# abhi1kumar/SUP-NeRF

Hardware: AMD Instinct MI355X
Metric: rays/sec at 4096 rays x 64 samples (fused render forward) (higher is better)
Workload: dtype f32

## Files before the change

### sup-nerf_amd/csrc/snr_mlp16.hip

```cpp
#include <atomic>

#include "snr_mlp16_core.hpp"
#include "snr_host.hpp"

namespace snr {

struct Epi {
    float lo;
    const float* zlds;
    const float* zglb;
    float hi;
    float* dump;
};
struct EpiRegs { f32x4 z; };

__device__ __forceinline__ uint32_t spread_nibbles(uint32_t m16) {
    return ((m16 >> 12) & 0xFu) | (((m16 >> 8) & 0xFu) << 8) | (((m16 >> 4) & 0xFu) << 16) | ((m16 & 0xFu) << 24);
}

template <bool LATLDS>
__device__ __forceinline__ EpiRegs epi_load(const Epi& c, int T, int g) {
    EpiRegs e;
    e.z = f32x4{0.f, 0.f, 0.f, 0.f};
    if (LATLDS) e.z = *reinterpret_cast<const f32x4*>(c.zlds + 16 * T + 4 * g);
    else if (c.zglb) e.z = *reinterpret_cast<const f32x4*>(c.zglb + 16 * T + 4 * g);
    return e;
}

template <bool MASKS>
__device__ __forceinline__ void epi_value(const f32x4& acc, f32x4& x, const Epi& c, const EpiRegs& e, int r, uint32_t& m16) {
    float v = acc[r];
    if (MASKS) m16 = __builtin_amdgcn_alignbit(m16, __float_as_uint(0.f - v), 31);
    v = __builtin_amdgcn_fmed3f(v, c.lo, c.hi);
    x[r] = v + e.z[r];
    if (MASKS) asm volatile("" : "+v"(m16));
}

template <int NT>
__device__ __forceinline__ void acc_from_bias(f32x4 (&acc)[16], const float* bias , int g) {
#pragma unroll
    for (int t = 0; t < NT; ++t) acc[t] = *reinterpret_cast<const f32x4*>(bias + 16 * t + 4 * g);
}

template <int NT, int WAVES, bool LATLDS, bool MASKS, bool DUMP>
__device__ __forceinline__ void layer_from_acc(f32x4 (&accP)[16], Ring16& ring, float* lds, const float* bias, const Epi& c, int g, const Dma16& dm,
                                               const float* base, bool pre, const f32x4 (&xe)[2], const float* next_first, int next_rows,
                                               uint32_t (&mw)[4]) {
    f32x4 accC[16];
    f32x4 a0, a1;
    constexpr int rows_mid = NT * 16;
    constexpr int chunk_floats = rows_mid * KC;
    if (pre) {
        chunk_dma16<WAVES>(dm, base, lds + (ring.cur ^ 1) * WBUF16, lds, rows_mid);
        const float* wb = lds + ring.cur * WBUF16;
        first_pair(a0, a1, wb + ring.aoff[0]);
        acc_from_bias<NT>(accC, bias, g);
        tile_mma<NT, false>(accC, accP, xe[0], wb + ring.aoff[0], a0, a1, wb + ring.aoff[1]);
        tile_mma<NT, false>(accC, accP, xe[1], wb + ring.aoff[1], a0, a1, nullptr);
        ring_turn(ring);
    } else {
        acc_from_bias<NT>(accC, bias, g);
    }
    constexpr int NG = NT / 2;
    EpiRegs e = epi_load<LATLDS>(c, 0, g);
    f32x4 xa, xb;
    uint32_t m16 = 0u;
#pragma unroll
    for (int r = 3; r >= 0; --r) epi_value<MASKS>(accP[0], xa, c, e, r, m16);
    if (DUMP) *reinterpret_cast<f32x4*>(c.dump) = xa;
#pragma unroll
    for (int ch = 0; ch < 8; ++ch) {
        const float* src = (ch < 7) ? base + (ch + 1) * chunk_floats : next_first;
        const int rows = (ch < 7) ? rows_mid : next_rows;
        float* const dst = lds + (ring.cur ^ 1) * WBUF16;
        const float* wb = lds + ring.cur * WBUF16;
        first_pair(a0, a1, wb + ring.aoff[0]);
        tile_mma<NT, false>(accC, accP, xa, wb + ring.aoff[0], a0, a1, wb + ring.aoff[1], [&](int gi) {
            if (gi == 0) e = epi_load<LATLDS>(c, 2 * ch + 1, g);
            constexpr int PSTEP = (WAVES == 8) ? 2 : 1;
            if (gi % PSTEP == 0 && (gi / PSTEP) * 8 * WAVES < rows) chunk_piece16<WAVES>(dm, src, dst, lds, rows, gi / PSTEP);
#pragma unroll
            for (int k = (gi * 4) / NG; k < ((gi + 1) * 4) / NG; ++k) epi_value<MASKS>(accP[2 * ch + 1], xb, c, e, 3 - k, m16);
            if (DUMP && gi == NG - 1) *reinterpret_cast<f32x4*>(c.dump + 16 * (2 * ch + 1)) = xb;
        });
        if (ch & 1) { mw[ch >> 1] = m16; m16 = 0u; }
        if (ch == 7) {
            tile_mma<NT, true>(accC, accP, xb, wb + ring.aoff[1], a0, a1, nullptr);
        } else {
            tile_mma<NT, false>(accC, accP, xb, wb + ring.aoff[1], a0, a1, nullptr, [&](int gi) {
                if (gi == 0) e = epi_load<LATLDS>(c, 2 * ch + 2, g);
#pragma unroll
                for (int k = (gi * 4) / NG; k < ((gi + 1) * 4) / NG; ++k) epi_value<MASKS>(accP[2 * ch + 2], xa, c, e, 3 - k, m16);
                if (DUMP && gi == NG - 1) *reinterpret_cast<f32x4*>(c.dump + 16 * (2 * ch + 2)) = xa;
            });
        }
        ring_turn(ring);
    }
}

__device__ __forceinline__ void store_masks16x4(uint4* __restrict__ dst , const uint32_t (&mw)[4], int wave, int lane) {
    const int n = lane & 15, g = lane >> 4;
    uint32_t w[4];
#pragma unroll
    for (int i = 0; i < 4; ++i) {
        const uint32_t mine = spread_nibbles(mw[i]) << (4 * (g >> 1));
        w[i] = mine | (uint32_t)__shfl_xor((int)mine, 32, 64);
    }
    if (g < 2) dst[16 * (wave & 1) + n + 32 * g] = make_uint4(w[0], w[1], w[2], w[3]);
}

#ifdef SNR_STAMPS
#define SNR16_STAMP(i) do { if (io.sigmas && lane == 0) { unsigned long long t_; asm volatile("s_memtime %0\n\ts_waitcnt lgkmcnt(0)" : "=s"(t_) :: "memory"); \
        reinterpret_cast<unsigned long long*>(io.sigmas)[(tile_wg * WAVES + wave) * 8 + (i)] = t_; } } while (0)
#define SNR16_STAMP_HWID(i) do { if (io.sigmas && lane == 0) { unsigned a_, b_; asm volatile("s_getreg_b32 %0, hwreg(HW_REG_HW_ID)\n\ts_getreg_b32 %1, hwreg(HW_REG_XCC_ID)" : "=s"(a_), "=s"(b_)); \
        reinterpret_cast<unsigned long long*>(io.sigmas)[(tile_wg * WAVES + wave) * 8 + (i)] = (unsigned long long)a_ | ((unsigned long long)b_ << 32); } } while (0)
#else
#define SNR16_STAMP(i) do {} while (0)
#define SNR16_STAMP_HWID(i) do {} while (0)
#endif

template <int MODE, int WAVES, bool LATLDS, bool MASKS, bool DUMP>
__global__ void __launch_bounds__(WAVES * 64, 2)
decoder_fwd16_kernel(DecoderIO io, Layout L, Lds16 lo, const float* __restrict__ xyz, const float* __restrict__ viewdir, RayGeom gm,
                     float* __restrict__ out_rgb, float* __restrict__ out_depth, float* __restrict__ out_acc) {
    extern __shared__ __attribute__((aligned(16))) float lds[];
    constexpr int WGP = WAVES * 16;
    const int tid = threadIdx.x, lane = tid & 63, wave = tid >> 6, n = lane & 15, g = lane >> 4;
    const long long tile_wg = blockIdx.x;
    const long long gp_raw = tile_wg * WGP + wave * 16 + n;
    const bool live = gp_raw < io.n_points;
    const long long gp = live ? gp_raw : io.n_points - 1;
    const long long tile32 = tile_wg * (WAVES / 2) + (wave >> 1);
    const bool tile_live = tile32 * 32 < io.n_points;
    const int sb = io.sb, tb = io.tb;
    const int n_relu = n_relu_layers(sb, tb);
    SNR16_STAMP(0);
    __builtin_amdgcn_s_setprio(3);
    float px, py, pz, dx, dy, dz, zc = 0.f;
    if (MODE == 0) {
        px = xyz[gp * 3]; py = xyz[gp * 3 + 1]; pz = xyz[gp * 3 + 2];
        dx = viewdir[gp * 3]; dy = viewdir[gp * 3 + 1]; dz = viewdir[gp * 3 + 2];
    } else {
        const PointId id = point_id(gm, tile_wg, WGP, wave * 16 + n, live);
        const SamplePoint sp = make_sample(gm, id.ray, id.s, id.obj);
        px = sp.x; py = sp.y; pz = sp.z; dx = sp.dx; dy = sp.dy; dz = sp.dz; zc = sp.zc;
    }
    const float* bias = lds + lo.bias;
    const float* heads = bias + L.n_mfma_layers * 256;
    const float* zero = lds + lo.zero;
    const float* lat_lane = io.latent + (gp / io.points_per_obj) * (long long)L.n_lat * 256;
    const float* lat_wg = io.latent + ((tile_wg * WGP) / io.points_per_obj) * (long long)L.n_lat * 256;

    Ring16 ring;
    ring.cur = 0;
    Dma16 dm;
    dm.voff = lane * 16u + 4096u;
    dm.lds0 = __builtin_amdgcn_readfirstlane((unsigned)(size_t)(__attribute__((address_space(3))) float*)lds);
    dm.wave = __builtin_amdgcn_readfirstlane(wave);
    {
        const int sw = (n >> 1) & 7;
        ring.aoff[0] = n * KC + (((0 + g) ^ sw) << 2);
        ring.aoff[1] = n * KC + (((4 + g) ^ sw) << 2);
    }
    constexpr long long C256 = 256 * KC;
    const int li_encshape = sb + 1, li_view = sb + 2, li_last = sb + tb + 2;
    const float* const stream = io.packed + L.fwd;
    auto layer_base = [&](int li) { return stream + 2 * C256 + (long long)(li - 1) * 8 * C256 + (li > li_view ? C256 : 0); };
    auto layer_first = [&](int li) { return layer_base(li) + (li == li_view ? 8 * C256 : 0); };
    f32x4 xin[4], xd[2];
    {
        chunk_dma16<WAVES>(dm, stream, lds, lds, 256);
        for (int r = dm.wave; r < L.n_mfma_layers + 3; r += WAVES) row_dma16(dm, io.packed + L.bias + r * 256, lds + lo.bias + r * 256, lds);
        if (LATLDS)
            for (int r = dm.wave; r < L.n_lat; r += WAVES) row_dma16(dm, lat_wg + r * 256, lds + lo.lat + r * 256, lds);
        if (tid < 64) *reinterpret_cast<f32x4*>(lds + lo.zero + 4 * tid) = f32x4{0.f, 0.f, 0.f, 0.f};
        float* sc = lds + lo.scratch + wave * PE_WAVE16 + n * PE_ROW;
#pragma unroll 1
        for (int i = 0; i < 8; i += 2) {
            const int q = 8 * g + i;
            if (q < 3 * XYZ_FREQ) {
                f32x2 sn, cs;
                pe_sincos2(f32x2{ldexpf(pick3(px, py, pz, q % 3), q / 3), ldexpf(pick3(px, py, pz, (q + 1) % 3), (q + 1) / 3)}, &sn, &cs);
                sc[3 + q] = sn[0]; sc[3 + 3 * XYZ_FREQ + q] = cs[0];
                sc[4 + q] = sn[1]; sc[4 + 3 * XYZ_FREQ + q] = cs[1];
            }
        }
        {
            const int q = 3 * g;
            f32x2 sn, cs;
            pe_sincos2(f32x2{ldexpf(pick3(dx, dy, dz, q % 3), q / 3), ldexpf(pick3(dx, dy, dz, (q + 1) % 3), (q + 1) / 3)}, &sn, &cs);
            sc[64 + 3 + q] = sn[0]; sc[64 + 3 + 3 * DIR_FREQ + q] = cs[0];
            sc[64 + 4 + q] = sn[1]; sc[64 + 4 + 3 * DIR_FREQ + q] = cs[1];
            float s1, c1;
            pe_sincos(ldexpf(pick3(dx, dy, dz, (q + 2) % 3), (q + 2) / 3), &s1, &c1);
            sc[64 + 5 + q] = s1; sc[64 + 5 + 3 * DIR_FREQ + q] = c1;
        }
        if (g == 0) {
            sc[0] = px; sc[1] = py; sc[2] = pz; sc[63] = 0.f;
            sc[64] = dx; sc[65] = dy; sc[66] = dz;
#pragma unroll
            for (int f = D_DIR; f < 32; ++f) sc[64 + f] = 0.f;
        }
        asm volatile("s_waitcnt vmcnt(0)" ::: "memory");
        __syncthreads();
#pragma unroll
        for (int T = 0; T < 4; ++T)
#pragma unroll
            for (int r = 0; r < 4; ++r) xin[T][r] = sc[16 * T + 4 * g + r];
#pragma unroll
        for (int T = 0; T < 2; ++T)
#pragma unroll
            for (int r = 0; r < 4; ++r) xd[T][r] = sc[64 + 16 * T + 4 * g + r];
        if (WAVES == 4) __syncthreads();
    }

    __builtin_amdgcn_s_setprio(0);
    SNR16_STAMP(1);
    f32x4 accP[16];
    {
        f32x4 accC[16];
        f32x4 a0, a1;
        acc_from_bias<16>(accC, bias, g);
#pragma unroll
        for (int ch = 0; ch < 2; ++ch) {
            chunk_dma16<WAVES>(dm, ch == 0 ? stream + C256 : layer_first(1), lds + (ring.cur ^ 1) * WBUF16, lds, 256);
            const float* wb = lds + ring.cur * WBUF16;
            first_pair(a0, a1, wb + ring.aoff[0]);
            tile_mma<16, false>(accC, accP, xin[2 * ch], wb + ring.aoff[0], a0, a1, wb + ring.aoff[1]);
            if (ch == 1) tile_mma<16, true>(accC, accP, xin[2 * ch + 1], wb + ring.aoff[1], a0, a1, nullptr);
            else tile_mma<16, false>(accC, accP, xin[2 * ch + 1], wb + ring.aoff[1], a0, a1, nullptr);
            ring_turn(ring);
        }
    }

    SNR16_STAMP(2);
    uint32_t mw[4] = {0u, 0u, 0u, 0u};
    float o_sigma = 0.f;
    float pos_inf = __builtin_inff();
    asm volatile("" : "+v"(pos_inf));
    float* const dump_lane = DUMP ? io.act + gp * 256 + 4 * g : nullptr;
    auto epi_of = [&](int lp) {
        const int la = latent_after(lp, sb, tb);
        Epi c;
        c.lo = (lp != li_encshape) ? 0.f : -__builtin_inff();
        c.zlds = (la >= 0) ? lds + lo.lat + la * 256 : zero;
        c.zglb = (la >= 0) ? lat_lane + la * 256 : nullptr;
        c.hi = pos_inf;
        c.dump = DUMP ? dump_lane + (long long)lp * io.n_points * 256 : nullptr;
        return c;
    };
    auto after_layer_input = [&](int lp) {
        if (MASKS && lp != li_encshape && tile_live) store_masks16x4(io.masks + (tile32 * n_relu + relu_slot(lp, sb)) * 64, mw, wave, lane);
    };
#pragma unroll 1
    for (int li = 1; li <= li_last; ++li) {
        const int lp = li - 1;
        const Epi c = epi_of(lp);
        if (li == li_view) {
            SNR16_STAMP(3);
            float s = 0.f;
#pragma unroll
            for (int T = 0; T < 16; ++T) {
                const f32x4 ws = *reinterpret_cast<const f32x4*>(heads + 16 * T + 4 * g);
#pragma unroll
                for (int r = 0; r < 4; ++r) s = fmaf(ws[r], accP[T][r], s);
            }
            s += __shfl_xor(s, 16, 64);
            s += __shfl_xor(s, 32, 64);
            const float pre = s + heads[L.sigma_b - L.sigma_w];
            o_sigma = pre > 20.f ? pre : log1pf(expf(pre));
        }
        layer_from_acc<16, WAVES, LATLDS, MASKS, DUMP>(accP, ring, lds, bias + li * 256, c, g, dm, layer_base(li), li == li_view, xd, layer_first(li + 1),
                                                       (li == li_last) ? 128 : 256, mw);
        after_layer_input(lp);
    }
    SNR16_STAMP(4);
    {
        const Epi c = epi_of(li_last);
        layer_from_acc<8, WAVES, LATLDS, MASKS, DUMP>(accP, ring, lds, bias + (li_last + 1) * 256, c, g, dm, layer_base(li_last + 1), false, xd, nullptr, 0, mw);
        after_layer_input(li_last);
    }

    SNR16_STAMP(5);
    __builtin_amdgcn_s_setprio(3);
    float o_r, o_g, o_b;
    {
        const float* w2 = heads + (L.rgb2_w - L.sigma_w);
        float pr = 0.f, pg = 0.f, pb = 0.f;
        uint32_t m16 = 0u, mr[4] = {0u, 0u, 0u, 0u};
        float* const dmp = DUMP ? dump_lane + (long long)(li_last + 1) * io.n_points * 256 : nullptr;
#pragma unroll
        for (int T = 0; T < 8; ++T) {
            const f32x4 wr = *reinterpret_cast<const f32x4*>(w2 + 16 * T + 4 * g);
            const f32x4 wg = *reinterpret_cast<const f32x4*>(w2 + 128 + 16 * T + 4 * g);
            const f32x4 wb = *reinterpret_cast<const f32x4*>(w2 + 256 + 16 * T + 4 * g);
            f32x4 xv;
#pragma unroll
            for (int r = 3; r >= 0; --r) {
                float v = accP[T][r];
                m16 = __builtin_amdgcn_alignbit(m16, __float_as_uint(0.f - v), 31);
                v = fmaxf(v, 0.f);
                xv[r] = v;
            }
#pragma unroll
            for (int r = 0; r < 4; ++r) { pr = fmaf(wr[r], xv[r], pr); pg = fmaf(wg[r], xv[r], pg); pb = fmaf(wb[r], xv[r], pb); }
            if (DUMP) *reinterpret_cast<f32x4*>(dmp + 16 * T) = xv;
            if ((T & 3) == 3) { mr[T >> 2] = m16; m16 = 0u; }
        }
        if (MASKS && tile_live) store_masks16x4(io.masks + (tile32 * n_relu + (n_relu - 1)) * 64, mr, wave, lane);
        pr += __shfl_xor(pr, 16, 64); pr += __shfl_xor(pr, 32, 64);
        pg += __shfl_xor(pg, 16, 64); pg += __shfl_xor(pg, 32, 64);
        pb += __shfl_xor(pb, 16, 64); pb += __shfl_xor(pb, 32, 64);
        const float* b2 = heads + (L.rgb2_b - L.sigma_w);
        o_r = pr + b2[0]; o_g = pg + b2[1]; o_b = pb + b2[2];
    }

    SNR16_STAMP_HWID(6);
#ifndef SNR_STAMPS
    if (live && g == 0 && io.sigmas) io.sigmas[gp] = o_sigma;
#endif
    if (live && g == 0) {
        if (io.rgbs) { io.rgbs[gp * 3] = o_r; io.rgbs[gp * 3 + 1] = o_g; io.rgbs[gp * 3 + 2] = o_b; }
    }
    if (MODE == 1) {
        float* comp = lds + lo.comp;
        if (g == 0) {
            float* c = comp + (wave * 16 + n) * COMP_STRIDE;
            c[0] = o_sigma; c[1] = o_r; c[2] = o_g; c[3] = o_b; c[4] = zc;
        }
        __syncthreads();
        const int S = gm.S;
        const int rays_here = WGP / S;
        const bool white = gm.flags & SNR_WHITE_BKGD;
        for (int r = wave; r < rays_here; r += WAVES) {
            const long long ray = tile_wg * rays_here + r;
            if (ray >= gm.n_rays) break;
            const float* c0 = comp + r * S * COMP_STRIDE;
            RayOut o = composite_ray_fwd(S, lane, white, [&](int k, float& s_, float& r_, float& g_, float& b_, float& z_, float& zn_) {
                const float* c = c0 + k * COMP_STRIDE;
                s_ = c[0]; r_ = c[1]; g_ = c[2]; b_ = c[3]; z_ = c[4];
                zn_ = (k < S - 1) ? c[COMP_STRIDE + 4] : 0.f;
            });
            if (lane == 0) {
                out_rgb[ray * 3] = o.r; out_rgb[ray * 3 + 1] = o.g; out_rgb[ray * 3 + 2] = o.b;
                out_depth[ray] = o.depth; out_acc[ray] = o.acc;
            }
        }
    }
    SNR16_STAMP(7);
}

}

using namespace snr;


template <int MODE, int WAVES, bool LATLDS, bool MASKS, bool DUMP>
static int launch16(const DecoderIO& io, const Layout& L, const Lds16& lo, const float* xyz, const float* viewdir, const RayGeom& g, float* rgb,
                    float* depth, float* acc, hipStream_t st) {
    auto kern = decoder_fwd16_kernel<MODE, WAVES, LATLDS, MASKS, DUMP>;
    static std::atomic<uint64_t> granted{0};
    int dev = 0;
    if (hipGetDevice(&dev) != hipSuccess) return SNR_E_LAUNCH;
    const uint64_t bit = dev < 64 ? (uint64_t)1 << dev : 0;
    if (!(granted.load(std::memory_order_acquire) & bit)) {
        if (hipFuncSetAttribute(reinterpret_cast<const void*>(kern), hipFuncAttributeMaxDynamicSharedMemorySize, 160 * 1024) != hipSuccess) return SNR_E_LAUNCH;
        granted.fetch_or(bit, std::memory_order_release);
    }
    const unsigned grid = (unsigned)((io.n_points + WAVES * 16 - 1) / (WAVES * 16));
    kern<<<grid, WAVES * 64, (size_t)lo.total * 4, st>>>(io, L, lo, xyz, viewdir, g, rgb, depth, acc);
    return snr_check_launch_();
}

template <int WAVES>
static int launch16_w(int mode, const DecoderIO& io, const Layout& L, const float* xyz, const float* viewdir, const RayGeom& g, float* rgb,
                      float* depth, float* acc, hipStream_t st) {
    const bool latlds = (io.points_per_obj % (WAVES * 16)) == 0 && L.n_lat <= LDS_LAT_ROWS;
    const bool masks = io.masks != nullptr;
    const Lds16 lo = make_lds16(WAVES, L.n_mfma_layers, latlds ? L.n_lat : LDS_LAT_ROWS + 1);
#define SNR_L16(M, LL, MK, DP) launch16<M, WAVES, LL, MK, DP>(io, L, lo, xyz, viewdir, g, rgb, depth, acc, st)
    if (mode == 0) {
        if (latlds) return masks ? SNR_L16(0, true, true, false) : SNR_L16(0, true, false, false);
        return masks ? SNR_L16(0, false, true, false) : SNR_L16(0, false, false, false);
    }
    if (latlds) return masks ? SNR_L16(1, true, true, false) : SNR_L16(1, true, false, false);
    return masks ? SNR_L16(1, false, true, false) : SNR_L16(1, false, false, false);
#undef SNR_L16
}

int snr_fp32_fwd16_launch_(int mode, const DecoderIO& io, const Layout& L, const float* xyz, const float* viewdir, const RayGeom& g, float* rgb,
                           float* depth, float* acc, void* stream_) {
    hipStream_t st = (hipStream_t)stream_;
    if (io.act) return SNR_E_UNSUPPORTED;
    const bool lat4 = (io.points_per_obj % 64) == 0 && L.n_lat <= LDS_LAT_ROWS;
    const Lds16 lo4 = make_lds16(4, L.n_mfma_layers, lat4 ? L.n_lat : LDS_LAT_ROWS + 1);
    const bool four = lo4.total * 4 <= 80 * 1024 && (mode == 0 || (g.S <= 64 && 64 % g.S == 0));
    return four ? launch16_w<4>(mode, io, L, xyz, viewdir, g, rgb, depth, acc, st) : launch16_w<8>(mode, io, L, xyz, viewdir, g, rgb, depth, acc, st);
}
```

### sup-nerf_amd/csrc/snr_mlp16_core.hpp

```cpp
#pragma once
#include "snr_mlp_core.hpp"

namespace snr {

constexpr int PE_WAVE16 = 16 * PE_ROW;
constexpr int WBUF16 = 256 * KC;

struct Lds16 { int ring1, scratch, comp, bias, lat, zero, total; };
inline Lds16 make_lds16(int waves, int n_mfma_layers, int n_lat) {
    Lds16 o;
    o.ring1 = WBUF16;
    int p = 2 * WBUF16;
    if (waves == 8) { o.scratch = p; p += 8 * PE_WAVE16; o.comp = p; p += 128 * COMP_STRIDE; }
    else { o.scratch = o.ring1; o.comp = 0; }
    p = (p + 3) & ~3;
    o.bias = p; p += (n_mfma_layers + 3) * 256;
    o.lat = p; p += (n_lat <= LDS_LAT_ROWS ? n_lat : 0) * 256;
    o.zero = p; p += 256;
    o.total = p;
    return o;
}

template <int K>
__device__ __forceinline__ void dma_piece_imm(unsigned voff, const void* sbase, unsigned m0v) {
    asm volatile("s_mov_b32 m0, %2\n\ts_nop 0\n\tglobal_load_lds_dwordx4 %0, %1 offset:%3" :: "v"(voff), "s"(sbase), "s"(m0v), "n"(1024 * K - 4096) : "memory");
}
__device__ __forceinline__ void dma_piece(int k, unsigned voff, const void* sbase, unsigned m0v) {
    switch (k) {
        case 0: dma_piece_imm<0>(voff, sbase, m0v); break;
        case 1: dma_piece_imm<1>(voff, sbase, m0v); break;
        case 2: dma_piece_imm<2>(voff, sbase, m0v); break;
        case 3: dma_piece_imm<3>(voff, sbase, m0v); break;
        case 4: dma_piece_imm<4>(voff, sbase, m0v); break;
        case 5: dma_piece_imm<5>(voff, sbase, m0v); break;
        case 6: dma_piece_imm<6>(voff, sbase, m0v); break;
        default: dma_piece_imm<7>(voff, sbase, m0v); break;
    }
}
struct Dma16 {
    unsigned voff;
    unsigned lds0;
    int wave;
};
template <int WAVES>
__device__ __forceinline__ void chunk_piece16(const Dma16& d, const float* __restrict__ g, const float* lds_dst, const float* lds_base, int rows, int i) {
    const unsigned sl = (unsigned)(rows * 128 / WAVES) * (unsigned)d.wave;
    const char* sbase = reinterpret_cast<const char*>(g) + sl;
    const unsigned m0v = __builtin_amdgcn_readfirstlane(d.lds0 + (unsigned)((lds_dst - lds_base) * 4) + sl + 4096u);
    dma_piece(i, d.voff, sbase, m0v);
}
template <int WAVES>
__device__ __forceinline__ void chunk_dma16(const Dma16& d, const float* __restrict__ g, const float* lds_dst, const float* lds_base, int rows) {
#pragma unroll
    for (int i = 0; i < 32 / WAVES; ++i)
        if (i * 8 * WAVES < rows) chunk_piece16<WAVES>(d, g, lds_dst, lds_base, rows, i);
}
__device__ __forceinline__ void row_dma16(const Dma16& d, const float* __restrict__ g, const float* lds_dst, const float* lds_base) {
    const unsigned m0v = __builtin_amdgcn_readfirstlane(d.lds0 + (unsigned)((lds_dst - lds_base) * 4) + 4096u);
    dma_piece_imm<0>(d.voff, g, m0v);
}

struct PointId { long long ray, obj; int s; };
__device__ __forceinline__ PointId point_id(const RayGeom& g, long long tile_wg, int wgp, int pl, bool live) {
    const int ls = 31 - __builtin_clz((unsigned)g.S);
    const long long ray0 = tile_wg * (long long)(wgp >> ls);
    const long long obj0 = ray0 / g.rays_per_obj;
    const long long rem0 = ray0 - obj0 * g.rays_per_obj;
    const int dr = pl >> ls;
    const long long r = rem0 + dr;
    PointId p;
    p.ray = ray0 + dr;
    p.s = pl & (g.S - 1);
    p.obj = obj0 + (g.rays_per_obj >= wgp ? (long long)(r >= g.rays_per_obj) : (long long)((unsigned)r / (unsigned)g.rays_per_obj));
    if (!live) { p.ray = g.n_rays - 1; p.s = g.S - 1; p.obj = (g.n_rays - 1) / g.rays_per_obj; }
    return p;
}

struct Ring16 {
    int cur;
    int aoff[2];
};

#define SNR16_WAIT_LDS() __builtin_amdgcn_s_waitcnt(0xc07f)

struct NoBetween { __device__ __forceinline__ void operator()(int) const {} };
constexpr int TM_LAST = 1, TM_ZERO = 2;
template <int NT, int FLAGS, class Between = NoBetween, int NA = 16, int ND = 16>
__device__ __forceinline__ void tile_mma(f32x4 (&accC)[NA], f32x4 (&accD)[ND], const f32x4& x, const float* wrow ,
                                         f32x4& a0, f32x4& a1, const float* wnext, Between&& between = NoBetween()) {
    constexpr bool LAST = FLAGS & TM_LAST, ZERO = FLAGS & TM_ZERO;
    const f32x4 zero4 = {0.f, 0.f, 0.f, 0.f};
#pragma unroll
    for (int t = 0; t < NT; t += 2) {
// ... 40 lines not shown
```

### sup-nerf_amd/csrc/snr_device.hpp

```cpp
#pragma once
#include <hip/hip_runtime.h>
#include "snr_layout.h"
#include "../../include/supnerf_hip.h"

namespace snr {

typedef float f32x4 __attribute__((ext_vector_type(4)));
typedef float f32x16 __attribute__((ext_vector_type(16)));

constexpr float LAST_DELTA = 1e10f;
constexpr float TRANS_EPS = 1e-10f;

__device__ __forceinline__ float sum_row_pairs(float v) {
    float a = v, b = v;
    asm volatile("s_nop 1\n\tv_permlane16_swap_b32 %0, %1" : "+v"(a), "+v"(b));
    return a + b;
}
__device__ __forceinline__ float sum_halves(float v) {
    float a = v, b = v;
    asm volatile("s_nop 1\n\tv_permlane32_swap_b32 %0, %1" : "+v"(a), "+v"(b));
    return a + b;
}

template <int CTRL>
// ... 111 lines not shown
    float zc;
    float t;
    float u;
};

__device__ __forceinline__ void philox4x32_10(unsigned long long key, unsigned long long ctr_lo, unsigned long long ctr_hi, uint32_t (&out)[4]) {
    uint32_t c0 = (uint32_t)ctr_lo, c1 = (uint32_t)(ctr_lo >> 32), c2 = (uint32_t)ctr_hi, c3 = (uint32_t)(ctr_hi >> 32);
    uint32_t k0 = (uint32_t)key, k1 = (uint32_t)(key >> 32);
#pragma unroll
    for (int r = 0; r < 10; ++r) {
        const uint32_t hi0 = __umulhi(0xD2511F53u, c0), lo0 = 0xD2511F53u * c0;
        const uint32_t hi1 = __umulhi(0xCD9E8D57u, c2), lo1 = 0xCD9E8D57u * c2;
        const uint32_t n0 = hi1 ^ c1 ^ k0, n2 = hi0 ^ c3 ^ k1;
        c0 = n0; c1 = lo1; c2 = n2; c3 = lo0;
        k0 += 0x9E3779B9u; k1 += 0xBB67AE85u;
    }
    out[0] = c0; out[1] = c1; out[2] = c2; out[3] = c3;
}

__device__ __forceinline__ float box_jitter_rng(const RayGeom& g, long long i) {
    unsigned long long sub = (unsigned long long)i, round = 0;
    int word = 0;
    if (g.rng_threads) {
        if ((((unsigned long long)i | (g.rng_threads << 2)) >> 32) == 0) {
            const uint32_t thr = (uint32_t)g.rng_threads, per_round = thr << 2, i32 = (uint32_t)i;
            const uint32_t rd = i32 / per_round, r = i32 - rd * per_round, w = r / thr;
            round = rd; word = (int)w; sub = r - w * thr;
        } else {
            const unsigned long long per_round = g.rng_threads * 4ull;
            round = (unsigned long long)i / per_round;
            const unsigned long long r = (unsigned long long)i - round * per_round;
            word = (int)(r / g.rng_threads);
            sub = r - (unsigned long long)word * g.rng_threads;
        }
    }
    uint32_t w[4];
    philox4x32_10(g.rng_seed, g.rng_offset / 4ull + round, sub, w);
    const uint32_t v = word == 0 ? w[0] : (word == 1 ? w[1] : (word == 2 ? w[2] : w[3]));
    const float f = __fadd_rn(2.3283064e-10f, __fmul_rn((float)v, 2.3283064e-10f));
    return f == 1.0f ? 0.f : f;
}

__device__ __forceinline__ float nan_min(float a, float b) { return (a != a || b != b) ? __builtin_nanf("") : fminf(a, b); }
__device__ __forceinline__ float nan_max(float a, float b) { return (a != a || b != b) ? __builtin_nanf("") : fmaxf(a, b); }

struct BoxSlab {
    float inv[3], tmin[3], tmax[3];
    float t_near, t_far;
    bool hit;
};
__device__ __forceinline__ BoxSlab box_slab(const float (&o)[3], const float (&d)[3], const float (&hb)[3]) {
    BoxSlab b;
#pragma unroll
    for (int a = 0; a < 3; ++a) {
        b.inv[a] = __fdiv_rn(1.f, d[a]);
        b.tmin[a] = __fmul_rn(__fsub_rn(-hb[a], o[a]), b.inv[a]);
        b.tmax[a] = __fmul_rn(__fsub_rn(hb[a], o[a]), b.inv[a]);
    }
    const float l0 = nan_min(b.tmin[0], b.tmax[0]), l1 = nan_min(b.tmin[1], b.tmax[1]), l2 = nan_min(b.tmin[2], b.tmax[2]);
    const float h0 = nan_max(b.tmin[0], b.tmax[0]), h1 = nan_max(b.tmin[1], b.tmax[1]), h2 = nan_max(b.tmin[2], b.tmax[2]);
    b.t_near = nan_max(nan_max(l0, l1), l2);
    b.t_far = nan_min(nan_min(h0, h1), h2);
    b.hit = (b.t_far > b.t_near) && (b.t_far > 0.f);
    return b;
}

__device__ __forceinline__ void box_ray(const RayGeom& g, long long ray, long long obj, float (&o)[3], float (&d)[3], float (&hb)[3], float& zs) {
    zs = g.z_scale[obj];
#pragma unroll
    for (int a = 0; a < 3; ++a) {
        o[a] = __fdiv_rn(g.rays_o[ray * 3 + a], zs);
        d[a] = g.rays_d[ray * 3 + a];
        hb[a] = g.box_half[obj * 3 + a];
    }
}

__device__ __forceinline__ void box_ray(const RayGeom& g, long long ray, float (&o)[3], float (&d)[3], float (&hb)[3], float& zs) {
    box_ray(g, ray, ray / g.rays_per_obj, o, d, hb, zs);
}

__device__ __forceinline__ float load_t(const RayGeom& g, long long ray, int s, long long obj) {
    long long idx = g.z_mode == SNR_Z_SHARED ? s : (g.z_mode == SNR_Z_PER_OBJECT ? obj * g.S + s : ray * g.S + s);
    return g.t_vals[idx];
}

__device__ __forceinline__ SamplePoint make_sample(const RayGeom& g, long long ray, int s, long long obj) {
    SamplePoint sp;
    float ox, oy, oz, t;
    const float dx = g.rays_d[ray * 3 + 0], dy = g.rays_d[ray * 3 + 1], dz = g.rays_d[ray * 3 + 2];
    const bool box = g.z_mode == SNR_Z_BOX;
    sp.u = 0.f;
    if (box) {
        float o[3], d[3], hb[3], zs;
        box_ray(g, ray, obj, o, d, hb, zs);
        const BoxSlab b = box_slab(o, d, hb);
        const float near = b.hit ? b.t_near : -1.f, far = b.hit ? b.t_far : -1.f;
        const float step = 1.f / (float)g.S;
        const float jit = g.t_vals ? g.t_vals[ray * g.S + s] : box_jitter_rng(g, ray * g.S + s);
        sp.u = __fadd_rn((float)s * step, __fmul_rn(jit, step));
        t = __fadd_rn(__fmul_rn(near, __fsub_rn(1.f, sp.u)), __fmul_rn(far, sp.u));
        ox = o[0]; oy = o[1]; oz = o[2];
    } else {
        ox = g.rays_o[ray * 3 + 0]; oy = g.rays_o[ray * 3 + 1]; oz = g.rays_o[ray * 3 + 2];
        t = load_t(g, ray, s, obj);
    }
    float px = __fadd_rn(ox, __fmul_rn(dx, t));
    float py = __fadd_rn(oy, __fmul_rn(dy, t));
    float pz = __fadd_rn(oz, __fmul_rn(dz, t));
    sp.t = t;
    if (g.flags & SNR_METRIC_Z) {
        const float zs = g.z_scale[obj];
        float ex = __fmul_rn(__fsub_rn(px, ox), zs), ey = __fmul_rn(__fsub_rn(py, oy), zs), ez = __fmul_rn(__fsub_rn(pz, oz), zs);
        sp.zc = sqrtf(__fmaf_rn(ez, ez, __fmaf_rn(ey, ey, __fmul_rn(ex, ex))));
    } else {
        sp.zc = t;
    }
    if (!box) {
        const float dv = g.xyz_div[obj];
        px = __fdiv_rn(px, dv); py = __fdiv_rn(py, dv); pz = __fdiv_rn(pz, dv);
    }
    px = __fmul_rn(px, g.xyz_mul);
    py = __fmul_rn(py, g.xyz_mul);
    pz = __fmul_rn(pz, g.xyz_mul);
    sp.x = g.m[0] * px + g.m[1] * py + g.m[2] * pz;
    sp.y = g.m[3] * px + g.m[4] * py + g.m[5] * pz;
    sp.z = g.m[6] * px + g.m[7] * py + g.m[8] * pz;
    sp.dx = g.m[0] * dx + g.m[1] * dy + g.m[2] * dz;
    sp.dy = g.m[3] * dx + g.m[4] * dy + g.m[5] * dz;
    sp.dz = g.m[6] * dx + g.m[7] * dy + g.m[8] * dz;
    return sp;
}
__device__ __forceinline__ SamplePoint make_sample(const RayGeom& g, long long ray, int s) { return make_sample(g, ray, s, ray / g.rays_per_obj); }

__device__ __forceinline__ float pick3(float a, float b, float c, int i) { return i == 0 ? a : (i == 1 ? b : c); }

struct RayOut { float r, g, b, depth, acc; };

template <class Fetch>
__device__ __forceinline__ RayOut composite_ray_fwd(int S, int lane, bool white, Fetch&& fetch) {
    float carry = 1.f;
    float sr = 0.f, sg = 0.f, sb = 0.f, sd = 0.f, sw = 0.f, acc = 0.f;
    for (int base = 0; base < S; base += 64) {
        const int k = base + lane;
        const bool valid = k < S;
        float sig = 0.f, cr = 0.f, cg = 0.f, cb = 0.f, z = 0.f, zn = 0.f;
        if (valid) fetch(k, sig, cr, cg, cb, z, zn);
        const float delta = (k == S - 1) ? LAST_DELTA : zn - z;
        const float alpha = 1.f - expf(-fmaxf(sig, 0.f) * delta);
        const float T = valid ? (1.f - alpha) + TRANS_EPS : 1.f;
        const float incl = wave_scan_mul(T, lane);
        const float excl = wave_shift_up1(incl, 1.f);
        const float A = carry * excl;
        const float w = valid ? alpha * A : 0.f;
        sr += w * cr; sg += w * cg; sb += w * cb; sd += w * z; sw += w;
        if (k == S - 1) acc = A;
        carry *= wave_lane(incl, 63);
    }
    RayOut o;
    o.r = wave_sum(sr); o.g = wave_sum(sg); o.b = wave_sum(sb); o.depth = wave_sum(sd);
    const float wsum = wave_sum(sw);
    o.acc = wave_lane(acc, (S - 1) & 63);
    if (white) { const float bg = 1.f - wsum; o.r += bg; o.g += bg; o.b += bg; }
    return o;
}

template <int NCH, class Fetch, class Emit>
__device__ __forceinline__ void composite_ray_bwd(int S, int lane, bool white, float g_r, float g_g, float g_b,
                                                  float g_depth, float g_acc, Fetch&& fetch, Emit&& emit) {
    float sig[NCH], cr[NCH], cg[NCH], cb[NCH], z[NCH], delta[NCH], e[NCH], T[NCH], A[NCH], w[NCH], dw[NCH];
    float carry = 1.f, acc_last = 0.f;
    const float g_white = white ? (g_r + g_g + g_b) : 0.f;
#pragma unroll
    for (int c = 0; c < NCH; ++c) {
        const int k = c * 64 + lane;
        const bool valid = k < S;
        float zn = 0.f;
        sig[c] = cr[c] = cg[c] = cb[c] = z[c] = 0.f;
        if (valid) fetch(k, sig[c], cr[c], cg[c], cb[c], z[c], zn);
        delta[c] = (k == S - 1) ? LAST_DELTA : zn - z[c];
        e[c] = expf(-fmaxf(sig[c], 0.f) * delta[c]);
        const float alpha = 1.f - e[c];
        T[c] = valid ? (1.f - alpha) + TRANS_EPS : 1.f;
        const float incl = wave_scan_mul(T[c], lane);
        const float excl = wave_shift_up1(incl, 1.f);
        A[c] = carry * excl;
        w[c] = valid ? alpha * A[c] : 0.f;
        dw[c] = valid ? (g_r * cr[c] + g_g * cg[c] + g_b * cb[c] + g_depth * z[c] - g_white) : 0.f;
        if (k == S - 1) acc_last = A[c];
        carry *= wave_lane(incl, 63);
    }
    acc_last = wave_lane(acc_last, (S - 1) & 63);
    float tail = 0.f;
    float dd[NCH];
#pragma unroll
    for (int c = NCH - 1; c >= 0; --c) {
        const int k = c * 64 + lane;
        const bool valid = k < S;
        const float p = dw[c] * w[c];
        const float incl = wave_suffix_sum(p, lane);
        const float R = (incl - p) + tail + ((k < S - 1) ? g_acc * acc_last : 0.f);
        tail += wave_lane(incl, 0);
        const float dT = R / T[c];
        const float dalpha = dw[c] * A[c] - dT;
        const float s = fmaxf(sig[c], 0.f);
        const float dsig = (valid && sig[c] > 0.f) ? dalpha * delta[c] * e[c] : 0.f;
        dd[c] = (valid && k < S - 1) ? dalpha * s * e[c] : 0.f;
        sig[c] = dsig;
    }
#pragma unroll
    for (int c = 0; c < NCH; ++c) {
        const int k = c * 64 + lane;
        const bool valid = k < S;
// ... 106 lines not shown
```

Measured before the change: 2.470 million.

## Compute view-direction layer term once per ray instead of per sample

In fused render mode, every sample on a ray shares the same view direction. The view-dependent input contribution to the view layer (bias plus weight times direction encoding) is now computed once per ray with scalar FMAs and stored in LDS. The layer then starts its accumulators from that per-ray vector instead of running the two direction MFMA chunks for each sample. The direction encoding is also spread across lanes per wave. In exchange the code adds LDS aliasing (it reuses scratch or bias space) and an extra sync path, and it only applies when the sample count is a multiple of 16.

```diff
diff --git a/sup-nerf_amd/csrc/snr_mlp16.hip b/sup-nerf_amd/csrc/snr_mlp16.hip
--- a/sup-nerf_amd/csrc/snr_mlp16.hip
+++ b/sup-nerf_amd/csrc/snr_mlp16.hip
@@ -42,15 +42,52 @@
     for (int t = 0; t < NT; ++t) acc[t] = *reinterpret_cast<const f32x4*>(bias + 16 * t + 4 * g);
 }
 
+struct RayStart { float* u; int r0, r1; };
+__device__ __forceinline__ void ray_start(const RayStart& rs, const float* bias, const float* wb , const f32x4 (&xe)[2],
+                                          int lane) {
+    float* const pe_lds = rs.u + rs.r0;
+    if ((lane & 15) == 0) {
+        *reinterpret_cast<f32x4*>(pe_lds + 4 * (lane >> 4)) = xe[0];
+        *reinterpret_cast<f32x4*>(pe_lds + 16 + 4 * (lane >> 4)) = xe[1];
+    }
+    f32x4 pe[2][4];
+#pragma unroll
+    for (int dT = 0; dT < 2; ++dT)
+#pragma unroll
+        for (int g = 0; g < 4; ++g) pe[dT][g] = *reinterpret_cast<const f32x4*>(pe_lds + 16 * dT + 4 * g);
+#pragma unroll 1
+    for (int row = rs.r0 + lane; row < rs.r1; row += 64) {
+        float acc = bias[row];
+        const float* w = wb + row * KC;
+        const int sw = (row >> 1) & 7;
+#pragma unroll
+        for (int dT = 0; dT < 2; ++dT) {
+            f32x4 a[4];
+#pragma unroll
+            for (int g = 0; g < 4; ++g) a[g] = *reinterpret_cast<const f32x4*>(w + (((4 * dT + g) ^ sw) << 2));
+#pragma unroll
+            for (int r = 0; r < 4; ++r)
+#pragma unroll
+                for (int g = 0; g < 4; ++g) acc = fmaf(a[g][r], pe[dT][g][r], acc);
+        }
+        rs.u[row] = acc;
+    }
+}
+
 template <int NT, int WAVES, bool LATLDS, bool MASKS, bool DUMP>
 __device__ __forceinline__ void layer_from_acc(f32x4 (&accP)[16], Ring16& ring, float* lds, const float* bias, const Epi& c, int g, const Dma16& dm,
-                                               const float* base, bool pre, const f32x4 (&xe)[2], const float* next_first, int next_rows,
-                                               uint32_t (&mw)[4]) {
+                                               const float* base, bool pre, const f32x4 (&xe)[2], const RayStart& rs, const float* next_first,
+                                               int next_rows, uint32_t (&mw)[4]) {
     f32x4 accC[16];
     f32x4 a0, a1;
     constexpr int rows_mid = NT * 16;
     constexpr int chunk_floats = rows_mid * KC;
-    if (pre) {
+    if (pre && rs.u) {
+        chunk_dma16<WAVES>(dm, base, lds + (ring.cur ^ 1) * WBUF16, lds, rows_mid);
+        ray_start(rs, bias, lds + ring.cur * WBUF16, xe, (int)(threadIdx.x & 63));
+        ring_turn(ring);
+        acc_from_bias<NT>(accC, rs.u, g);
+    } else if (pre) {
         chunk_dma16<WAVES>(dm, base, lds + (ring.cur ^ 1) * WBUF16, lds, rows_mid);
         const float* wb = lds + ring.cur * WBUF16;
         first_pair(a0, a1, wb + ring.aoff[0]);
@@ -134,6 +171,7 @@
     const bool tile_live = tile32 * 32 < io.n_points;
     const int sb = io.sb, tb = io.tb;
     const int n_relu = n_relu_layers(sb, tb);
+    const bool raydir = MODE == 1 && lo.ray >= 0;
     SNR16_STAMP(0);
     __builtin_amdgcn_s_setprio(3);
     float px, py, pz, dx, dy, dz, zc = 0.f;
@@ -185,7 +223,18 @@
                 sc[4 + q] = sn[1]; sc[4 + 3 * XYZ_FREQ + q] = cs[1];
             }
         }
-        {
+        float* const sd = raydir ? lds + lo.scratch + wave * PE_WAVE16 + 64 : sc + 64;
+        if (raydir) {
+            if (lane < 3 * DIR_FREQ) {
+                float s1, c1;
+                pe_sincos(ldexpf(pick3(dx, dy, dz, lane % 3), lane / 3), &s1, &c1);
+                sd[3 + lane] = s1; sd[3 + 3 * DIR_FREQ + lane] = c1;
+            } else if (lane < 3 * DIR_FREQ + 3) {
+                sd[lane - 3 * DIR_FREQ] = pick3(dx, dy, dz, lane - 3 * DIR_FREQ);
+            } else if (lane >= D_DIR && lane < 32) {
+                sd[lane] = 0.f;
+            }
+        } else {
             const int q = 3 * g;
             f32x2 sn, cs;
             pe_sincos2(f32x2{ldexpf(pick3(dx, dy, dz, q % 3), q / 3), ldexpf(pick3(dx, dy, dz, (q + 1) % 3), (q + 1) / 3)}, &sn, &cs);
@@ -194,13 +243,13 @@
             float s1, c1;
             pe_sincos(ldexpf(pick3(dx, dy, dz, (q + 2) % 3), (q + 2) / 3), &s1, &c1);
             sc[64 + 5 + q] = s1; sc[64 + 5 + 3 * DIR_FREQ + q] = c1;
-        }
-        if (g == 0) {
-            sc[0] = px; sc[1] = py; sc[2] = pz; sc[63] = 0.f;
-            sc[64] = dx; sc[65] = dy; sc[66] = dz;
-#pragma unroll
-            for (int f = D_DIR; f < 32; ++f) sc[64 + f] = 0.f;
-        }
+            if (g == 0) {
+                sc[64] = dx; sc[65] = dy; sc[66] = dz;
+#pragma unroll
+                for (int f = D_DIR; f < 32; ++f) sc[64 + f] = 0.f;
+            }
+        }
+        if (g == 0) { sc[0] = px; sc[1] = py; sc[2] = pz; sc[63] = 0.f; }
         asm volatile("s_waitcnt vmcnt(0)" ::: "memory");
         __syncthreads();
 #pragma unroll
@@ -210,7 +259,7 @@
 #pragma unroll
         for (int T = 0; T < 2; ++T)
 #pragma unroll
-            for (int r = 0; r < 4; ++r) xd[T][r] = sc[64 + 16 * T + 4 * g + r];
+            for (int r = 0; r < 4; ++r) xd[T][r] = sd[16 * T + 4 * g + r];
         if (WAVES == 4) __syncthreads();
     }
 
@@ -235,6 +284,13 @@
 
     SNR16_STAMP(2);
     uint32_t mw[4] = {0u, 0u, 0u, 0u};
+    RayStart rs{nullptr, 0, 0};
+    if (raydir) {
+        const int lw = __builtin_ctz((unsigned)gm.S) - 4;
+        rs.u = lds + lo.ray + (dm.wave >> lw) * 256;
+        rs.r0 = (dm.wave & ((1 << lw) - 1)) * (256 >> lw);
+        rs.r1 = rs.r0 + (256 >> lw);
+    }
     float o_sigma = 0.f;
     float pos_inf = __builtin_inff();
     asm volatile("" : "+v"(pos_inf));
@@ -270,14 +326,14 @@
             const float pre = s + heads[L.sigma_b - L.sigma_w];
             o_sigma = pre > 20.f ? pre : log1pf(expf(pre));
         }
-        layer_from_acc<16, WAVES, LATLDS, MASKS, DUMP>(accP, ring, lds, bias + li * 256, c, g, dm, layer_base(li), li == li_view, xd, layer_first(li + 1),
+        layer_from_acc<16, WAVES, LATLDS, MASKS, DUMP>(accP, ring, lds, bias + li * 256, c, g, dm, layer_base(li), li == li_view, xd, rs, layer_first(li + 1),
                                                        (li == li_last) ? 128 : 256, mw);
         after_layer_input(lp);
     }
     SNR16_STAMP(4);
     {
         const Epi c = epi_of(li_last);
-        layer_from_acc<8, WAVES, LATLDS, MASKS, DUMP>(accP, ring, lds, bias + (li_last + 1) * 256, c, g, dm, layer_base(li_last + 1), false, xd, nullptr, 0, mw);
+        layer_from_acc<8, WAVES, LATLDS, MASKS, DUMP>(accP, ring, lds, bias + (li_last + 1) * 256, c, g, dm, layer_base(li_last + 1), false, xd, rs, nullptr, 0, mw);
         after_layer_input(li_last);
     }
 
@@ -377,7 +433,8 @@
                       float* depth, float* acc, hipStream_t st) {
     const bool latlds = (io.points_per_obj % (WAVES * 16)) == 0 && L.n_lat <= LDS_LAT_ROWS;
     const bool masks = io.masks != nullptr;
-    const Lds16 lo = make_lds16(WAVES, L.n_mfma_layers, latlds ? L.n_lat : LDS_LAT_ROWS + 1);
+    Lds16 lo = make_lds16(WAVES, L.n_mfma_layers, latlds ? L.n_lat : LDS_LAT_ROWS + 1);
+    if (mode == 1 && g.S % 16 == 0 && (WAVES == 8 || WAVES * 16 / g.S <= L.sb + 2)) lo.ray = WAVES == 8 ? lo.scratch : lo.bias;
 #define SNR_L16(M, LL, MK, DP) launch16<M, WAVES, LL, MK, DP>(io, L, lo, xyz, viewdir, g, rgb, depth, acc, st)
     if (mode == 0) {
         if (latlds) return masks ? SNR_L16(0, true, true, false) : SNR_L16(0, true, false, false);
diff --git a/sup-nerf_amd/csrc/snr_mlp16_core.hpp b/sup-nerf_amd/csrc/snr_mlp16_core.hpp
--- a/sup-nerf_amd/csrc/snr_mlp16_core.hpp
+++ b/sup-nerf_amd/csrc/snr_mlp16_core.hpp
@@ -6,9 +6,10 @@
 constexpr int PE_WAVE16 = 16 * PE_ROW;
 constexpr int WBUF16 = 256 * KC;
 
-struct Lds16 { int ring1, scratch, comp, bias, lat, zero, total; };
+struct Lds16 { int ring1, scratch, comp, bias, lat, zero, total, ray; };
 inline Lds16 make_lds16(int waves, int n_mfma_layers, int n_lat) {
     Lds16 o;
+    o.ray = -1;
     o.ring1 = WBUF16;
     int p = 2 * WBUF16;
     if (waves == 8) { o.scratch = p; p += 8 * PE_WAVE16; o.comp = p; p += 128 * COMP_STRIDE; }
```

Result: faster. 2.507 million (median of 6 runs) (+1.5%).

## Precompute per-ray view-direction layer term once per ray in LDS

Applied to the files above, without the earlier changes.

In ray mode, the view-direction positional encoding is now computed once per ray instead of once per sample. Its contribution to the view layer (direction weights times encoding plus bias) is computed with a few MFMAs and stored in LDS as a per-ray seed. The view layer then starts from that seed instead of the bias and skips the direction chunk of its matmul. This adds LDS usage, extra template variants and a preload of the direction weights into registers, which may raise register pressure.

```diff
diff --git a/sup-nerf_amd/csrc/snr_device.hpp b/sup-nerf_amd/csrc/snr_device.hpp
--- a/sup-nerf_amd/csrc/snr_device.hpp
+++ b/sup-nerf_amd/csrc/snr_device.hpp
@@ -217,6 +217,15 @@
 __device__ __forceinline__ float load_t(const RayGeom& g, long long ray, int s, long long obj) {
     long long idx = g.z_mode == SNR_Z_SHARED ? s : (g.z_mode == SNR_Z_PER_OBJECT ? obj * g.S + s : ray * g.S + s);
     return g.t_vals[idx];
+}
+
+__device__ __forceinline__ void frame_dir(const RayGeom& g, float dx, float dy, float dz, float& ox, float& oy, float& oz) {
+    ox = g.m[0] * dx + g.m[1] * dy + g.m[2] * dz;
+    oy = g.m[3] * dx + g.m[4] * dy + g.m[5] * dz;
+    oz = g.m[6] * dx + g.m[7] * dy + g.m[8] * dz;
+}
+__device__ __forceinline__ void ray_frame_dir(const RayGeom& g, long long ray, float& ox, float& oy, float& oz) {
+    frame_dir(g, g.rays_d[ray * 3 + 0], g.rays_d[ray * 3 + 1], g.rays_d[ray * 3 + 2], ox, oy, oz);
 }
 
 __device__ __forceinline__ SamplePoint make_sample(const RayGeom& g, long long ray, int s, long long obj) {
@@ -260,9 +269,7 @@
     sp.x = g.m[0] * px + g.m[1] * py + g.m[2] * pz;
     sp.y = g.m[3] * px + g.m[4] * py + g.m[5] * pz;
     sp.z = g.m[6] * px + g.m[7] * py + g.m[8] * pz;
-    sp.dx = g.m[0] * dx + g.m[1] * dy + g.m[2] * dz;
-    sp.dy = g.m[3] * dx + g.m[4] * dy + g.m[5] * dz;
-    sp.dz = g.m[6] * dx + g.m[7] * dy + g.m[8] * dz;
+    frame_dir(g, dx, dy, dz, sp.dx, sp.dy, sp.dz);
     return sp;
 }
 __device__ __forceinline__ SamplePoint make_sample(const RayGeom& g, long long ray, int s) { return make_sample(g, ray, s, ray / g.rays_per_obj); }
diff --git a/sup-nerf_amd/csrc/snr_mlp16.hip b/sup-nerf_amd/csrc/snr_mlp16.hip
--- a/sup-nerf_amd/csrc/snr_mlp16.hip
+++ b/sup-nerf_amd/csrc/snr_mlp16.hip
@@ -119,10 +119,11 @@
 #define SNR16_STAMP_HWID(i) do {} while (0)
 #endif
 
-template <int MODE, int WAVES, bool LATLDS, bool MASKS, bool DUMP>
+template <int MODE, int WAVES, bool LATLDS, bool MASKS, bool DUMP, bool SEED = false>
 __global__ void __launch_bounds__(WAVES * 64, 2)
 decoder_fwd16_kernel(DecoderIO io, Layout L, Lds16 lo, const float* __restrict__ xyz, const float* __restrict__ viewdir, RayGeom gm,
-                     float* __restrict__ out_rgb, float* __restrict__ out_depth, float* __restrict__ out_acc) {
+                     float* __restrict__ out_rgb, float* __restrict__ out_depth, float* __restrict__ out_acc, int seed) {
+    static_assert(!SEED || MODE == 1, "the per-ray direction term needs rays");
     extern __shared__ __attribute__((aligned(16))) float lds[];
     constexpr int WGP = WAVES * 16;
     const int tid = threadIdx.x, lane = tid & 63, wave = tid >> 6, n = lane & 15, g = lane >> 4;
@@ -166,8 +167,20 @@
     const int li_encshape = sb + 1, li_view = sb + 2, li_last = sb + tb + 2;
     const float* const stream = io.packed + L.fwd;
     auto layer_base = [&](int li) { return stream + 2 * C256 + (long long)(li - 1) * 8 * C256 + (li > li_view ? C256 : 0); };
-    auto layer_first = [&](int li) { return layer_base(li) + (li == li_view ? 8 * C256 : 0); };
-    f32x4 xin[4], xd[2];
+    auto layer_first = [&](int li) { return layer_base(li) + (!SEED && li == li_view ? 8 * C256 : 0); };
+    const int ls = MODE == 1 ? 31 - __builtin_clz((unsigned)gm.S) : 0;
+    const int rays_wg = MODE == 1 ? WGP >> ls : 0;
+    constexpr int SEED_T = 16 / WAVES;
+    f32x4 xin[4], xd[2], va[SEED ? SEED_T : 1][2];
+    if (SEED) {
+        const float* vchunk = layer_base(li_view) + 8 * C256;
+        const int sw = (n >> 1) & 7;
+#pragma unroll
+        for (int j = 0; j < SEED_T; ++j)
+#pragma unroll
+            for (int T = 0; T < 2; ++T)
+                va[j][T] = *reinterpret_cast<const f32x4*>(vchunk + (16 * (SEED_T * wave + j) + n) * KC + (((4 * T + g) ^ sw) << 2));
+    }
     {
         chunk_dma16<WAVES>(dm, stream, lds, lds, 256);
         for (int r = dm.wave; r < L.n_mfma_layers + 3; r += WAVES) row_dma16(dm, io.packed + L.bias + r * 256, lds + lo.bias + r * 256, lds);
@@ -185,32 +198,65 @@
                 sc[4 + q] = sn[1]; sc[4 + 3 * XYZ_FREQ + q] = cs[1];
             }
         }
-        {
-            const int q = 3 * g;
+        float* sd = sc + 64;
+        int gq = g;
+        bool dir_here = true;
+        if (SEED) {
+            const int rho = lane >> 2;
+            gq = lane & 3;
+            dir_here = wave == 0 && rho < rays_wg;
+            sd = lds + lo.scratch + rho * PE_ROW + 64;
+            if (dir_here) {
+                const long long ray = tile_wg * rays_wg + rho;
+                ray_frame_dir(gm, ray < gm.n_rays ? ray : gm.n_rays - 1, dx, dy, dz);
+            }
+        }
+        if (dir_here) {
+            const int q = 3 * gq;
             f32x2 sn, cs;
             pe_sincos2(f32x2{ldexpf(pick3(dx, dy, dz, q % 3), q / 3), ldexpf(pick3(dx, dy, dz, (q + 1) % 3), (q + 1) / 3)}, &sn, &cs);
-            sc[64 + 3 + q] = sn[0]; sc[64 + 3 + 3 * DIR_FREQ + q] = cs[0];
-            sc[64 + 4 + q] = sn[1]; sc[64 + 4 + 3 * DIR_FREQ + q] = cs[1];
+            sd[3 + q] = sn[0]; sd[3 + 3 * DIR_FREQ + q] = cs[0];
+            sd[4 + q] = sn[1]; sd[4 + 3 * DIR_FREQ + q] = cs[1];
             float s1, c1;
             pe_sincos(ldexpf(pick3(dx, dy, dz, (q + 2) % 3), (q + 2) / 3), &s1, &c1);
-            sc[64 + 5 + q] = s1; sc[64 + 5 + 3 * DIR_FREQ + q] = c1;
-        }
-        if (g == 0) {
-            sc[0] = px; sc[1] = py; sc[2] = pz; sc[63] = 0.f;
-            sc[64] = dx; sc[65] = dy; sc[66] = dz;
-#pragma unroll
-            for (int f = D_DIR; f < 32; ++f) sc[64 + f] = 0.f;
-        }
+            sd[5 + q] = s1; sd[5 + 3 * DIR_FREQ + q] = c1;
+            if (gq == 0) {
+                sd[0] = dx; sd[1] = dy; sd[2] = dz;
+#pragma unroll
+                for (int f = D_DIR; f < 32; ++f) sd[f] = 0.f;
+            }
+        }
+        if (g == 0) { sc[0] = px; sc[1] = py; sc[2] = pz; sc[63] = 0.f; }
         asm volatile("s_waitcnt vmcnt(0)" ::: "memory");
         __syncthreads();
 #pragma unroll
         for (int T = 0; T < 4; ++T)
 #pragma unroll
             for (int r = 0; r < 4; ++r) xin[T][r] = sc[16 * T + 4 * g + r];
-#pragma unroll
-        for (int T = 0; T < 2; ++T)
-#pragma unroll
-            for (int r = 0; r < 4; ++r) xd[T][r] = sc[64 + 16 * T + 4 * g + r];
+        if (SEED) {
+            const float* sdn = lds + lo.scratch + n * PE_ROW + 64;
+#pragma unroll
+            for (int T = 0; T < 2; ++T)
+#pragma unroll
+                for (int r = 0; r < 4; ++r) xd[T][r] = sdn[16 * T + 4 * g + r];
+            f32x4 sacc[SEED_T];
+#pragma unroll
+            for (int j = 0; j < SEED_T; ++j) sacc[j] = *reinterpret_cast<const f32x4*>(bias + li_view * 256 + 16 * (SEED_T * wave + j) + 4 * g);
+#pragma unroll
+            for (int T = 0; T < 2; ++T)
+#pragma unroll
+                for (int r = 0; r < 4; ++r)
+#pragma unroll
+                    for (int j = 0; j < SEED_T; ++j) sacc[j] = __builtin_amdgcn_mfma_f32_16x16x4f32(va[j][T][r], xd[T][r], sacc[j], 0, 0, 0);
+            if (n < rays_wg)
+#pragma unroll
+                for (int j = 0; j < SEED_T; ++j) *reinterpret_cast<f32x4*>(lds + seed + n * 256 + 16 * (SEED_T * wave + j) + 4 * g) = sacc[j];
+        } else {
+#pragma unroll
+            for (int T = 0; T < 2; ++T)
+#pragma unroll
+                for (int r = 0; r < 4; ++r) xd[T][r] = sc[64 + 16 * T + 4 * g + r];
+        }
         if (WAVES == 4) __syncthreads();
     }
 
@@ -270,7 +316,8 @@
             const float pre = s + heads[L.sigma_b - L.sigma_w];
             o_sigma = pre > 20.f ? pre : log1pf(expf(pre));
         }
-        layer_from_acc<16, WAVES, LATLDS, MASKS, DUMP>(accP, ring, lds, bias + li * 256, c, g, dm, layer_base(li), li == li_view, xd, layer_first(li + 1),
+        const float* start = (SEED && li == li_view) ? lds + seed + ((wave * 16 + n) >> ls) * 256 : bias + li * 256;
+        layer_from_acc<16, WAVES, LATLDS, MASKS, DUMP>(accP, ring, lds, start, c, g, dm, layer_base(li), !SEED && li == li_view, xd, layer_first(li + 1),
                                                        (li == li_last) ? 128 : 256, mw);
         after_layer_input(lp);
     }
@@ -355,10 +402,10 @@
 using namespace snr;
 
 
-template <int MODE, int WAVES, bool LATLDS, bool MASKS, bool DUMP>
+template <int MODE, int WAVES, bool LATLDS, bool MASKS, bool DUMP, bool SEED = false>
 static int launch16(const DecoderIO& io, const Layout& L, const Lds16& lo, const float* xyz, const float* viewdir, const RayGeom& g, float* rgb,
-                    float* depth, float* acc, hipStream_t st) {
-    auto kern = decoder_fwd16_kernel<MODE, WAVES, LATLDS, MASKS, DUMP>;
+                    float* depth, float* acc, hipStream_t st, int seed = 0) {
+    auto kern = decoder_fwd16_kernel<MODE, WAVES, LATLDS, MASKS, DUMP, SEED>;
     static std::atomic<uint64_t> granted{0};
     int dev = 0;
     if (hipGetDevice(&dev) != hipSuccess) return SNR_E_LAUNCH;
@@ -368,7 +415,7 @@
         granted.fetch_or(bit, std::memory_order_release);
     }
     const unsigned grid = (unsigned)((io.n_points + WAVES * 16 - 1) / (WAVES * 16));
-    kern<<<grid, WAVES * 64, (size_t)lo.total * 4, st>>>(io, L, lo, xyz, viewdir, g, rgb, depth, acc);
+    kern<<<grid, WAVES * 64, (size_t)lo.total * 4, st>>>(io, L, lo, xyz, viewdir, g, rgb, depth, acc, seed);
     return snr_check_launch_();
 }
 
@@ -377,14 +424,28 @@
                       float* depth, float* acc, hipStream_t st) {
     const bool latlds = (io.points_per_obj % (WAVES * 16)) == 0 && L.n_lat <= LDS_LAT_ROWS;
     const bool masks = io.masks != nullptr;
-    const Lds16 lo = make_lds16(WAVES, L.n_mfma_layers, latlds ? L.n_lat : LDS_LAT_ROWS + 1);
+    Lds16 lo = make_lds16(WAVES, L.n_mfma_layers, latlds ? L.n_lat : LDS_LAT_ROWS + 1);
 #define SNR_L16(M, LL, MK, DP) launch16<M, WAVES, LL, MK, DP>(io, L, lo, xyz, viewdir, g, rgb, depth, acc, st)
+#define SNR_L16S(LL, MK) launch16<1, WAVES, LL, MK, false, true>(io, L, lo, xyz, viewdir, g, rgb, depth, acc, st, seed)
     if (mode == 0) {
         if (latlds) return masks ? SNR_L16(0, true, true, false) : SNR_L16(0, true, false, false);
         return masks ? SNR_L16(0, false, true, false) : SNR_L16(0, false, false, false);
     }
+    const int rays = WAVES * 16 / g.S;
+    int seed = -1;
+    if (rays == 1) {
+        seed = lo.bias + (io.sb + 2) * 256;
+    } else if (rays <= 16 && (lo.total + rays * 256) * 4 <= WAVES * 20 * 1024) {
+        seed = lo.total;
+        lo.total += rays * 256;
+    }
+    if (seed >= 0) {
+        if (latlds) return masks ? SNR_L16S(true, true) : SNR_L16S(true, false);
+        return masks ? SNR_L16S(false, true) : SNR_L16S(false, false);
+    }
     if (latlds) return masks ? SNR_L16(1, true, true, false) : SNR_L16(1, true, false, false);
     return masks ? SNR_L16(1, false, true, false) : SNR_L16(1, false, false, false);
+#undef SNR_L16S
 #undef SNR_L16
 }
 
```

Result: faster. 2.470 million before, 2.500 million after (median of 6 runs) (+1.2%).
